# Gorilla-Lab-SCUT/GeoA3

Hardware: AMD Instinct MI355X
Metric: attack-iterations/sec (B=250, N=1024) (higher is better)
Workload: dtype f32; 1 GPU; configs[1]: PointNet 1024-pt, 250 instances sharded over 1 GPU(s) (250 on rank 0), full GeoA3 (CE + CD 1.0 + HD 0.1 + curvature 1.0 k=16), untargeted; instances_per_gpu=250, global_batch=250, npoint=1024, knn=16, classes=40, wide_mode=f16x2, presteps=150, parallelism=instance-sharded x1

## Files before the change

geoa3_amd/csrc/pointnet_wide_bwdconv.hip:

```cpp
#include "pointnet_kernels.h"
#include <type_traits>

namespace {

constexpr int WM_CI = 128;

constexpr int BW2_WAVES = 8, BW2_THREADS = 64 * BW2_WAVES;
#ifdef GEOA3_BC_STAMPS
__device__ unsigned long long g_bc_stamps[3 * 8 * 16];
#define BC_STAMP(i)                                                                                          \
  do {                                                                                                       \
    if (tid == 0 && blockIdx.x == 5 && (blockIdx.y & 31) == 7 && blockIdx.y < 256)                            \
      g_bc_stamps[((TAPS == 3 ? 2 : (GF ? 1 : 0)) * 8 + (blockIdx.y >> 5)) * 16 + (i)] = __builtin_amdgcn_s_memtime(); \
  } while (0)
#else
#define BC_STAMP(i)
#endif
constexpr int BC_PT = WM_CI + 4;
template <int TAPS, bool GF = false, bool PRE = false>
__device__ __forceinline__ void wide_bwd_conv_body(const WideBwdArgs& a) {
  extern __shared__ __attribute__((aligned(16))) float smem[];
  constexpr int COLS = 64;
  float* s_acc = smem;
  int* s_flat = reinterpret_cast<int*>(smem);
  float* s_fg = smem + a.Co * TAPS;
  const int region = max(COLS * BC_PT, 2 * a.Co * TAPS);
  using list_t = typename std::conditional<TAPS == 1, uint16_t, int>::type;
  constexpr int LSH = TAPS == 1 ? 10 : 16;
  list_t* s_list = reinterpret_cast<list_t*>(smem + region);
  int* s_off = reinterpret_cast<int*>(smem + region) + (PRE ? 0 : (TAPS == 1 ? a.Co / 2 : a.Co * TAPS));
  int* s_wcnt = s_off + COLS + 1;
  int* s_sidecol = s_wcnt + BW2_WAVES + 1;
  float* s_side = reinterpret_cast<float*>(s_sidecol + BW2_WAVES);
  float* s_mx = s_side + BW2_WAVES * WM_CI;
  const int tid = threadIdx.x, lane = tid & 63, b = blockIdx.y, m0 = blockIdx.x * COLS;
  const int wave = __builtin_amdgcn_readfirstlane(tid >> 6);
  unsigned long long gw2 = 0ull;
  if (!GF && wave < 4) gw2 = a.Zmask2[((size_t)b * ((a.N + 63) >> 6) + blockIdx.x) * 64 + lane];
  const int tiles = (a.N + 63) >> 6;
  const ulonglong2 mkw = reinterpret_cast<const ulonglong2*>(a.Zmask + ((size_t)b * tiles + blockIdx.x) * WM_CI)[lane];
  const int qt = wave & 1, qc = (wave >> 1) & 1;

  float4* s_w1 = reinterpret_cast<float4*>((reinterpret_cast<uintptr_t>(s_side) + 15) & ~(uintptr_t)15);
  const float* gb = a.g + (size_t)b * a.Co;
  const int* argb = a.arg + (size_t)b * a.Co;
  const unsigned long long lt = (1ull << lane) - 1ull;
  BC_STAMP(0);
  constexpr int U = 8;
  const int* seg = nullptr;
  int ev0 = 0;
  if constexpr (PRE) {
    const int* ho = a.hoff + (size_t)b * (a.N + 1);
    const int h0 = ho[m0], h1 = ho[min(m0 + COLS, a.N)], hv = ho[min(m0 + min(tid, COLS), a.N)];
    seg = a.hits + (size_t)b * a.Co * TAPS + h0;
    {
      const int tot = h1 - h0, per = (tot + BW2_WAVES - 1) / BW2_WAVES;
      const int lo = min(tot, wave * per), hi = min(tot, lo + per);
      if (lo < hi) ev0 = seg[min(lo + (lane & (U - 1)), hi - 1)];
    }
    for (int e = tid; e < COLS * BC_PT; e += BW2_THREADS) s_acc[e] = 0.f;
    if (tid <= COLS) s_off[tid] = hv - h0;
    BC_STAMP(1);
    __syncthreads();
    BC_STAMP(2);
  } else {
  if (tid <= COLS) s_off[tid] = 0;
  __syncthreads();
  {
  const int cpw = (a.Co + BW2_WAVES - 1) / BW2_WAVES, c_lo = wave * cpw, c_hi = min(a.Co, c_lo + cpw);
  constexpr int MAXCH = 2;
  float gch[MAXCH];
  int bch[MAXCH];
  const bool regs = cpw <= 64 * MAXCH;
#pragma unroll
  for (int ch = 0; ch < MAXCH; ++ch) {
    const int co = c_lo + 64 * ch + lane;
    const bool in = regs && co < c_hi;
    gch[ch] = in ? gb[co] : 0.f;
    bch[ch] = (in ? argb[co] : 0) - TAPS / 2 - m0;
  }
  {
    int cnt = 0;
    int chn = 0;
    for (int c0 = c_lo; c0 < c_hi; c0 += 64, ++chn) {
      const int co = c0 + lane;
      const bool in = co < c_hi;
      const float g = regs ? (chn == 0 ? gch[0] : gch[1]) : (in ? gb[co] : 0.f);
      const int base = regs ? (chn == 0 ? bch[0] : bch[1]) : ((in ? argb[co] : 0) - TAPS / 2 - m0);
#pragma unroll
      for (int tap = 0; tap < TAPS; ++tap) {
        const int c = base + tap;
        const bool hit = g != 0.f && c >= 0 && c < COLS && m0 + c < a.N;
        cnt += __popcll(__ballot(hit));
        if (hit) atomicAdd(&s_off[c], 1);
      }
    }
    if (lane == 0) s_wcnt[wave] = cnt;
  }
  __syncthreads();
  if (tid == 0) {
    int run = 0;
    for (int w = 0; w < BW2_WAVES; ++w) {
      const int c = s_wcnt[w];
      s_wcnt[w] = run;
      run += c;
    }
    s_wcnt[BW2_WAVES] = run;
  }
  if (tid >= 64 && tid < 128) {
    const int cnt = s_off[lane];
    int incl = cnt;
#pragma unroll
    for (int o = 1; o < 64; o <<= 1) {
      const int v = __shfl_up(incl, o, 64);
      if (lane >= o) incl += v;
    }
    s_off[lane] = incl - cnt;
    if (lane == 63) s_off[COLS] = incl;
  }
  __syncthreads();
  {
    int pos = s_wcnt[wave];
    int chn = 0;
    for (int c0 = c_lo; c0 < c_hi; c0 += 64, ++chn) {
      const int co = c0 + lane;
      const bool in = co < c_hi;
      const float g = regs ? (chn == 0 ? gch[0] : gch[1]) : (in ? gb[co] : 0.f);
      const int base = regs ? (chn == 0 ? bch[0] : bch[1]) : ((in ? argb[co] : 0) - TAPS / 2 - m0);
#pragma unroll
      for (int tap = 0; tap < TAPS; ++tap) {
        const int c = base + tap;
        const bool hit = g != 0.f && c >= 0 && c < COLS && m0 + c < a.N;
        const unsigned long long mask = __ballot(hit);
        if (hit) {
          const int slot = pos + __popcll(mask & lt);
          s_flat[slot] = (co * TAPS + tap) | (c << 16);
          s_fg[slot] = g;
        }
        pos += __popcll(mask);
      }
    }
  }
  __syncthreads();
  }
  const int total = s_off[COLS];
  {
    int basec[COLS / BW2_WAVES];
#pragma unroll
    for (int j = 0; j < COLS / BW2_WAVES; ++j) basec[j] = s_off[(COLS / BW2_WAVES) * wave + j];
    for (int i0 = 0; i0 < total; i0 += 64) {
      const int i = i0 + lane;
      const int e = i < total ? s_flat[i] : -1;
      const int col = e >> 16;
#pragma unroll
      for (int j = 0; j < COLS / BW2_WAVES; ++j) {
        const bool mine = col == (COLS / BW2_WAVES) * wave + j;
        const unsigned long long mask = __ballot(mine);
        if (mine) {
          const int slot = basec[j] + __popcll(mask & lt);
          s_list[slot] = TAPS == 1 ? (list_t)((e & 0xffff) | ((e >> 16) << LSH)) : (list_t)e;
        }
        basec[j] += __popcll(mask);
      }
    }
  }
  __syncthreads();
  for (int e = tid; e < COLS * BC_PT; e += BW2_THREADS) s_acc[e] = 0.f;
  __syncthreads();
  }
  const int total = s_off[COLS];
  {
    const int per = (total + BW2_WAVES - 1) / BW2_WAVES;
    const int lo = min(total, wave * per), hi = min(total, lo + per);
    const int ldW = a.ldW ? a.ldW : WM_CI;
    int cur = -1;
    float acc0 = 0.f, acc1 = 0.f;
    auto load_ev = [&](int h0) -> int {
      const int i = min(h0 + (lane & (U - 1)), hi - 1);
      if constexpr (PRE) return seg[i];
      else return (int)s_list[i];
    };
    auto dec = [&](int e) -> int {
      if constexpr (PRE) return (e & 0xffff) | (((e >> 16) - m0) << LSH);
      else return e;
    };
    int evn = 0;
    if (lo < hi) evn = PRE ? ev0 : load_ev(lo);
    int side_col = -1;
    if (lo < hi) {
      const int c0 = dec(__builtin_amdgcn_readlane(evn, 0)) >> LSH;
      if (lo > s_off[c0]) side_col = c0;
    }
    bool in_side = side_col >= 0;
    auto flush = [&]() {
      if (cur < 0) return;
      if (in_side) {
        s_side[wave * WM_CI + 2 * lane] = acc0;
        s_side[wave * WM_CI + 2 * lane + 1] = acc1;
        in_side = false;
      } else {
        *reinterpret_cast<float2*>(s_acc + cur * BC_PT + 2 * lane) = make_float2(acc0, acc1);
      }
    };
    for (int h0 = lo; h0 < hi; h0 += U) {
      float2 w[U];
      float gg[U];
      int cc[U];
      const int ev = evn;
      if (h0 + U < hi) evn = load_ev(h0 + U);
#pragma unroll
      for (int u = 0; u < U; ++u) {
        const bool ok = h0 + u < hi;
        const int e = dec(__builtin_amdgcn_readlane(ev, u));
        const int er = e & ((1 << LSH) - 1);
        w[u] = *reinterpret_cast<const float2*>(a.W + (size_t)er * ldW + 2 * lane);
        gg[u] = ok ? gb[er / TAPS] : 0.f;
        cc[u] = ok ? e >> LSH : -2;
      }
#pragma unroll
      for (int u = 0; u < U; ++u) {
        if (cc[u] == -2) break;
        if (cc[u] != cur) {
          flush();
          cur = cc[u];
          acc0 = 0.f;
          acc1 = 0.f;
        }
        acc0 += w[u].x * gg[u];
        acc1 += w[u].y * gg[u];
      }
    }
    flush();
    if (lane == 0) s_sidecol[wave] = side_col;
    BC_STAMP(3);
  }
  __syncthreads();
  BC_STAMP(4);
  if (tid < WM_CI) {
    for (int w = 1; w < BW2_WAVES; ++w) {
      const int c = s_sidecol[w];
      if (c >= 0) s_acc[c * BC_PT + tid] += s_side[w * WM_CI + tid];
    }
  }
  __syncthreads();
  BC_STAMP(5);
  if (GF && tid < 64) s_w1[tid] = make_float4(a.w1[3 * tid], a.w1[3 * tid + 1], a.w1[3 * tid + 2], a.b1[tid]);
  float tv[16];
  {
    float mx = 0.f;
#pragma unroll
    for (int j = 0; j < 8; ++j) {
      const int c = 8 * wave + j;
      const float2 v = *reinterpret_cast<const float2*>(s_acc + c * BC_PT + 2 * lane);
      const bool in = m0 + c < a.N;
      tv[2 * j] = ((mkw.x >> c) & 1ull) && in ? v.x : 0.f;
      tv[2 * j + 1] = ((mkw.y >> c) & 1ull) && in ? v.y : 0.f;
      mx = fmaxf(mx, fmaxf(__builtin_fabsf(tv[2 * j]), __builtin_fabsf(tv[2 * j + 1])));
    }
    mx = wave_max(mx);
    if (lane == 0) s_mx[wave] = mx;
  }
  __syncthreads();
  BC_STAMP(6);
  float tm = s_mx[0];
#pragma unroll
  for (int w = 1; w < BW2_WAVES; ++w) tm = fmaxf(tm, s_mx[w]);
  const unsigned Ex = sf_exp(tm);
  const float sx = sf_scale(Ex);
  constexpr int BC_PH = 2 * BC_PT;
  _Float16* s_img = reinterpret_cast<_Float16*>(s_acc);
#pragma unroll
  for (int j = 0; j < 8; ++j) {
    const float x0 = tv[2 * j] * sx, x1 = tv[2 * j + 1] * sx;
    const _Float16 h0 = (_Float16)x0, h1 = (_Float16)x1;
    _Float16* row = s_img + (8 * wave + j) * BC_PH + 2 * lane;
    *reinterpret_cast<half2v*>(row) = half2v{h0, h1};
    *reinterpret_cast<half2v*>(row + WM_CI) = half2v{(_Float16)(x0 - (float)h0), (_Float16)(x1 - (float)h1)};
  }
  __syncthreads();
  if (wave >= 4) return;
  f32x16 acc;
#pragma unroll
  for (int r = 0; r < 16; ++r) acc[r] = 0.f;
  const _Float16* brow = s_img + (32 * qc + (lane & 31)) * BC_PH + (lane >> 5) * 8;
  {
    const half8* wf = reinterpret_cast<const half8*>(a.W2th) + (size_t)qt * 8 * 2 * 64 + lane;
    constexpr int WQ = 2;
    half8 wq[WQ][2];
#pragma unroll
    for (int c = 0; c + 1 < WQ; ++c) {
      wq[c][0] = wf[(2 * c) * 64];
      wq[c][1] = wf[(2 * c + 1) * 64];
    }
#pragma unroll
    for (int c = 0; c < 8; ++c) {
      if (c + WQ - 1 < 8) {
        wq[(c + WQ - 1) % WQ][0] = wf[(2 * (c + WQ - 1)) * 64];
        wq[(c + WQ - 1) % WQ][1] = wf[(2 * (c + WQ - 1) + 1) * 64];
      }
      const half8 wh = wq[c % WQ][0], wl = wq[c % WQ][1];
      const half8 xh = *reinterpret_cast<const half8*>(brow + c * 16);
      const half8 xl = *reinterpret_cast<const half8*>(brow + WM_CI + c * 16);
      acc = __builtin_amdgcn_mfma_f32_32x32x16_f16(wh, xh, acc, 0, 0, 0);
      acc = __builtin_amdgcn_mfma_f32_32x32x16_f16(wh, xl, acc, 0, 0, 0);
      acc = __builtin_amdgcn_mfma_f32_32x32x16_f16(wl, xh, acc, 0, 0, 0);
    }
  }
  BC_STAMP(7);
  const float un = sf_unscale(Ex) * a.w2th_unscale;
  const int col = 32 * qc + (lane & 31), m = m0 + col;
  if constexpr (GF) {
    const int ln = (int)__builtin_amdgcn_mbcnt_hi(~0u, __builtin_amdgcn_mbcnt_lo(~0u, 0u));
    const int mq = m0 + 32 * qc + (ln & 31);
    const bool in = mq < a.N;
    const float* xp = a.x3 + (size_t)b * 3 * a.N + (in ? mq : a.N - 1);
    const float x0 = xp[0], x1 = xp[a.N], x2 = xp[2 * (size_t)a.N];
    float q0 = 0.f, q1 = 0.f, q2 = 0.f;
#pragma unroll
    for (int r = 0; r < 16; ++r) {
      const float4 w = s_w1[32 * qt + (r & 3) + 8 * (r >> 2) + 4 * (ln >> 5)];
      const float o = (w.x * x0 + w.y * x1 + w.z * x2 + w.w) > 0.f ? acc[r] * un : 0.f;
      q0 += w.x * o;
      q1 += w.y * o;
      q2 += w.z * o;
    }
    q0 += __shfl_xor(q0, 32, 64);
    q1 += __shfl_xor(q1, 32, 64);
    q2 += __shfl_xor(q2, 32, 64);
    float4* s_q = s_w1 + 64;
    __syncthreads();
    if (qt == 1 && ln < 32) s_q[qc * 32 + ln] = make_float4(q0, q1, q2, 0.f);
    __syncthreads();
    if (qt == 0 && ln < 32 && in) {
      const float4 o = s_q[qc * 32 + ln];
      float* dxp = a.dx3 + (size_t)b * 3 * a.N + mq;
      dxp[0] += q0 + o.x;
      dxp[a.N] += q1 + o.y;
      dxp[2 * (size_t)a.N] += q2 + o.z;
    }
    BC_STAMP(8);
    return;
  }
  float* Y = a.dY + (size_t)b * a.sYb + m;
#pragma unroll
  for (int r = 0; r < 16; ++r) {
    const int rr = 32 * qt + (r & 3) + 8 * (r >> 2);
    const unsigned g0 = qc ? (unsigned)__builtin_amdgcn_readlane((int)(unsigned)(gw2 >> 32), rr)
                           : (unsigned)__builtin_amdgcn_readlane((int)(unsigned)gw2, rr);
    const unsigned g1 = qc ? (unsigned)__builtin_amdgcn_readlane((int)(unsigned)(gw2 >> 32), rr + 4)
                           : (unsigned)__builtin_amdgcn_readlane((int)(unsigned)gw2, rr + 4);
    const unsigned gsel = lane < 32 ? g0 : g1;
    const int row = rr + 4 * (lane >> 5);
    if (m < a.N) Y[(size_t)row * a.ldY] = (gsel >> (lane & 31)) & 1u ? acc[r] * un : 0.f;
  }
  BC_STAMP(8);
}

template <int TAPS, bool PRE>
__global__ __launch_bounds__(BW2_THREADS) void wide_bwd_conv_kernel(WideBwdArgs a) {
  wide_bwd_conv_body<TAPS, false, PRE>(a);
}
template <bool PRE>
__global__ __launch_bounds__(BW2_THREADS) __attribute__((amdgpu_waves_per_eu(8, 8))) void wide_bwd_conv_first_kernel(WideBwdArgs a) {
  wide_bwd_conv_body<1, true, PRE>(a);
}

}

#ifdef GEOA3_BC_STAMPS
extern "C" int geoa3_debug_bc_stamps(unsigned long long* out) {
  return hipMemcpyFromSymbol(out, HIP_SYMBOL(g_bc_stamps), sizeof(g_bc_stamps)) == hipSuccess ? 0 : -1;
}
#endif
int launch_wide_bwd_conv(const WideBwdArgs& a, hipStream_t s) {
  const bool gf = a.dx3 != nullptr;
  if ((a.taps != 1 && a.taps != 3) || !a.Zmask || !a.W2th || a.Co * a.taps > 0xffff || (a.taps == 1 && a.Co > 1024) ||
      (gf ? (!a.x3 || !a.w1 || !a.b1 || a.taps != 1) : (!a.Zmask2 || !a.dY)))
    return GEOA3_ENOSUPPORT;
  dim3 grid((a.N + 63) / 64, a.B);
  const size_t region = (size_t)64 * BC_PT > 2 * (size_t)a.Co * a.taps ? (size_t)64 * BC_PT : 2 * (size_t)a.Co * a.taps;
  const bool pre = a.hits && a.hoff;
  const size_t lds = (region + (pre ? 0 : (a.taps == 1 ? (size_t)a.Co / 2 : (size_t)a.Co * a.taps)) + 65 + 2 * BW2_WAVES + 1 + BW2_WAVES * WM_CI + 16 + 3 + 4) * sizeof(float);
  auto go = [&](auto kern) {
    (void)hipFuncSetAttribute(reinterpret_cast<const void*>(kern), hipFuncAttributeMaxDynamicSharedMemorySize, (int)lds);
    hipLaunchKernelGGL(kern, grid, dim3(BW2_THREADS), lds, s, a);
  };
  if (a.taps == 1 && a.dx3) pre ? go(wide_bwd_conv_first_kernel<true>) : go(wide_bwd_conv_first_kernel<false>);
  else if (a.taps == 1) pre ? go(wide_bwd_conv_kernel<1, true>) : go(wide_bwd_conv_kernel<1, false>);
  else pre ? go(wide_bwd_conv_kernel<3, true>) : go(wide_bwd_conv_kernel<3, false>);
  GEOA3_CHECK_LAUNCH();
  return GEOA3_OK;
}
```

Measured before the change: 650.4 iterations/s of a 250-instance batch.

## Software-pipeline backward-conv hit gathers and prefetch MFMA weights before barriers

The scatter-accumulate loop now loads 64 hit events per lane at once, gathers their gradient values in one load, and double-buffers the weight-row fetches in groups of 8 so loads overlap the accumulation. W2th MFMA operands, the Zmask2 word, the x3 coordinates and the w1 weights are prefetched before the reduction barriers, and the prefetch depth grows to 3 with sched_barrier ordering. The dx3 read is hoisted ahead of the reduction, and the non-first kernel gets waves_per_eu(8,8). This hides global-memory latency behind the barriers and compute, at the cost of more live registers that the occupancy attribute could force into spills.

```diff
diff --git a/geoa3_amd/csrc/pointnet_wide_bwdconv.hip b/geoa3_amd/csrc/pointnet_wide_bwdconv.hip
--- a/geoa3_amd/csrc/pointnet_wide_bwdconv.hip
+++ b/geoa3_amd/csrc/pointnet_wide_bwdconv.hip
@@ -35,20 +35,22 @@
   float* s_mx = s_side + BW2_WAVES * WM_CI;
   const int tid = threadIdx.x, lane = tid & 63, b = blockIdx.y, m0 = blockIdx.x * COLS;
   const int wave = __builtin_amdgcn_readfirstlane(tid >> 6);
-  unsigned long long gw2 = 0ull;
-  if (!GF && wave < 4) gw2 = a.Zmask2[((size_t)b * ((a.N + 63) >> 6) + blockIdx.x) * 64 + lane];
   const int tiles = (a.N + 63) >> 6;
   const ulonglong2 mkw = reinterpret_cast<const ulonglong2*>(a.Zmask + ((size_t)b * tiles + blockIdx.x) * WM_CI)[lane];
   const int qt = wave & 1, qc = (wave >> 1) & 1;
 
-  float4* s_w1 = reinterpret_cast<float4*>((reinterpret_cast<uintptr_t>(s_side) + 15) & ~(uintptr_t)15);
+  float4* s_w1 = reinterpret_cast<float4*>(smem + (((int)(s_side - smem) + 3) & ~3));
   const float* gb = a.g + (size_t)b * a.Co;
   const int* argb = a.arg + (size_t)b * a.Co;
   const unsigned long long lt = (1ull << lane) - 1ull;
   BC_STAMP(0);
-  constexpr int U = 8;
+  constexpr int U = 8, NB = 2, CH = 64;
   const int* seg = nullptr;
   int ev0 = 0;
+  float4 w1v = make_float4(0.f, 0.f, 0.f, 0.f);
+  if constexpr (GF) {
+    if (tid < 64) w1v = make_float4(a.w1[3 * tid], a.w1[3 * tid + 1], a.w1[3 * tid + 2], a.b1[tid]);
+  }
   if constexpr (PRE) {
     const int* ho = a.hoff + (size_t)b * (a.N + 1);
     const int h0 = ho[m0], h1 = ho[min(m0 + COLS, a.N)], hv = ho[min(m0 + min(tid, COLS), a.N)];
@@ -56,7 +58,7 @@
     {
       const int tot = h1 - h0, per = (tot + BW2_WAVES - 1) / BW2_WAVES;
       const int lo = min(tot, wave * per), hi = min(tot, lo + per);
-      if (lo < hi) ev0 = seg[min(lo + (lane & (U - 1)), hi - 1)];
+      if (lo < hi) ev0 = seg[min(lo + lane, hi - 1)];
     }
     for (int e = tid; e < COLS * BC_PT; e += BW2_THREADS) s_acc[e] = 0.f;
     if (tid <= COLS) s_off[tid] = hv - h0;
@@ -175,8 +177,8 @@
     const int ldW = a.ldW ? a.ldW : WM_CI;
     int cur = -1;
     float acc0 = 0.f, acc1 = 0.f;
-    auto load_ev = [&](int h0) -> int {
-      const int i = min(h0 + (lane & (U - 1)), hi - 1);
+    auto load_ev = [&](int c0) -> int {
+      const int i = min(c0 + lane, hi - 1);
       if constexpr (PRE) return seg[i];
       else return (int)s_list[i];
     };
@@ -202,49 +204,80 @@
         *reinterpret_cast<float2*>(s_acc + cur * BC_PT + 2 * lane) = make_float2(acc0, acc1);
       }
     };
-    for (int h0 = lo; h0 < hi; h0 += U) {
-      float2 w[U];
-      float gg[U];
-      int cc[U];
-      const int ev = evn;
-      if (h0 + U < hi) evn = load_ev(h0 + U);
-#pragma unroll
-      for (int u = 0; u < U; ++u) {
-        const bool ok = h0 + u < hi;
-        const int e = dec(__builtin_amdgcn_readlane(ev, u));
-        const int er = e & ((1 << LSH) - 1);
-        w[u] = *reinterpret_cast<const float2*>(a.W + (size_t)er * ldW + 2 * lane);
-        gg[u] = ok ? gb[er / TAPS] : 0.f;
-        cc[u] = ok ? e >> LSH : -2;
-      }
-#pragma unroll
-      for (int u = 0; u < U; ++u) {
-        if (cc[u] == -2) break;
-        if (cc[u] != cur) {
-          flush();
-          cur = cc[u];
-          acc0 = 0.f;
-          acc1 = 0.f;
+    for (int c0 = lo; c0 < hi; c0 += CH) {
+      const int ed = dec(evn);
+      const float gv = gb[(ed & ((1 << LSH) - 1)) / TAPS];
+      if (c0 + CH < hi) evn = load_ev(c0 + CH);
+      float2 w[NB][U];
+      auto request = [&](int k, float2 (&wk)[U]) {
+#pragma unroll
+        for (int u = 0; u < U; ++u) {
+          const int er = __builtin_amdgcn_readlane(ed, U * k + u) & ((1 << LSH) - 1);
+          wk[u] = *reinterpret_cast<const float2*>(a.W + (size_t)er * ldW + 2 * lane);
         }
-        acc0 += w[u].x * gg[u];
-        acc1 += w[u].y * gg[u];
+      };
+      auto consume = [&](int k, const float2 (&wk)[U]) {
+#pragma unroll
+        for (int u = 0; u < U; ++u) {
+          if (c0 + U * k + u >= hi) break;
+          const int c = __builtin_amdgcn_readlane(ed, U * k + u) >> LSH;
+          const float g = __int_as_float(__builtin_amdgcn_readlane(__float_as_int(gv), U * k + u));
+          if (c != cur) {
+            flush();
+            cur = c;
+            acc0 = 0.f;
+            acc1 = 0.f;
+          }
+          acc0 += wk[u].x * g;
+          acc1 += wk[u].y * g;
+        }
+      };
+#pragma unroll
+      for (int k = 0; k < CH / U + NB - 1; ++k) {
+        if (k < CH / U && c0 + U * k < hi) request(k, w[k % NB]);
+        if (k >= NB - 1) {
+          const int j = k - (NB - 1);
+          if (c0 + U * j >= hi) break;
+          consume(j, w[j % NB]);
+        }
       }
     }
     flush();
     if (lane == 0) s_sidecol[wave] = side_col;
     BC_STAMP(3);
   }
+  constexpr int WQ = 3;
+  const half8* wf = reinterpret_cast<const half8*>(a.W2th) + (size_t)qt * 8 * 2 * 64 + lane;
+  half8 wq[WQ][2];
+  unsigned long long gw2 = 0ull;
+  float x0 = 0.f, x1 = 0.f, x2 = 0.f;
+  if (wave < 4) {
+    if constexpr (!GF) gw2 = a.Zmask2[((size_t)b * tiles + blockIdx.x) * 64 + lane];
+#pragma unroll
+    for (int c = 0; c < WQ; ++c) {
+      wq[c][0] = wf[(2 * c) * 64];
+      wq[c][1] = wf[(2 * c + 1) * 64];
+    }
+    if constexpr (GF) {
+      const float* xp = a.x3 + (size_t)b * 3 * a.N + min(m0 + 32 * qc + (lane & 31), a.N - 1);
+      x0 = xp[0], x1 = xp[a.N], x2 = xp[2 * (size_t)a.N];
+    }
+  }
   __syncthreads();
   BC_STAMP(4);
   if (tid < WM_CI) {
+    int sc[BW2_WAVES];
+#pragma unroll
+    for (int w = 1; w < BW2_WAVES; ++w) sc[w] = s_sidecol[w];
+#pragma unroll
     for (int w = 1; w < BW2_WAVES; ++w) {
-      const int c = s_sidecol[w];
+      const int c = sc[w];
       if (c >= 0) s_acc[c * BC_PT + tid] += s_side[w * WM_CI + tid];
     }
   }
   __syncthreads();
   BC_STAMP(5);
-  if (GF && tid < 64) s_w1[tid] = make_float4(a.w1[3 * tid], a.w1[3 * tid + 1], a.w1[3 * tid + 2], a.b1[tid]);
+  if (GF && tid < 64) s_w1[tid] = w1v;
   float tv[16];
   {
     float mx = 0.f;
@@ -278,32 +311,24 @@
     *reinterpret_cast<half2v*>(row + WM_CI) = half2v{(_Float16)(x0 - (float)h0), (_Float16)(x1 - (float)h1)};
   }
   __syncthreads();
+  BC_STAMP(9);
   if (wave >= 4) return;
   f32x16 acc;
 #pragma unroll
   for (int r = 0; r < 16; ++r) acc[r] = 0.f;
   const _Float16* brow = s_img + (32 * qc + (lane & 31)) * BC_PH + (lane >> 5) * 8;
-  {
-    const half8* wf = reinterpret_cast<const half8*>(a.W2th) + (size_t)qt * 8 * 2 * 64 + lane;
-    constexpr int WQ = 2;
-    half8 wq[WQ][2];
-#pragma unroll
-    for (int c = 0; c + 1 < WQ; ++c) {
-      wq[c][0] = wf[(2 * c) * 64];
-      wq[c][1] = wf[(2 * c + 1) * 64];
-    }
-#pragma unroll
-    for (int c = 0; c < 8; ++c) {
-      if (c + WQ - 1 < 8) {
-        wq[(c + WQ - 1) % WQ][0] = wf[(2 * (c + WQ - 1)) * 64];
-        wq[(c + WQ - 1) % WQ][1] = wf[(2 * (c + WQ - 1) + 1) * 64];
-      }
-      const half8 wh = wq[c % WQ][0], wl = wq[c % WQ][1];
-      const half8 xh = *reinterpret_cast<const half8*>(brow + c * 16);
-      const half8 xl = *reinterpret_cast<const half8*>(brow + WM_CI + c * 16);
-      acc = __builtin_amdgcn_mfma_f32_32x32x16_f16(wh, xh, acc, 0, 0, 0);
-      acc = __builtin_amdgcn_mfma_f32_32x32x16_f16(wh, xl, acc, 0, 0, 0);
-      acc = __builtin_amdgcn_mfma_f32_32x32x16_f16(wl, xh, acc, 0, 0, 0);
+#pragma unroll
+  for (int c = 0; c < 8; ++c) {
+    const half8 wh = wq[c % WQ][0], wl = wq[c % WQ][1];
+    const half8 xh = *reinterpret_cast<const half8*>(brow + c * 16);
+    const half8 xl = *reinterpret_cast<const half8*>(brow + WM_CI + c * 16);
+    acc = __builtin_amdgcn_mfma_f32_32x32x16_f16(wh, xh, acc, 0, 0, 0);
+    acc = __builtin_amdgcn_mfma_f32_32x32x16_f16(wh, xl, acc, 0, 0, 0);
+    acc = __builtin_amdgcn_mfma_f32_32x32x16_f16(wl, xh, acc, 0, 0, 0);
+    if (c + WQ < 8) {
+      wq[c % WQ][0] = wf[(2 * (c + WQ)) * 64];
+      wq[c % WQ][1] = wf[(2 * (c + WQ) + 1) * 64];
+      __builtin_amdgcn_sched_barrier(0);
     }
   }
   BC_STAMP(7);
@@ -313,8 +338,9 @@
     const int ln = (int)__builtin_amdgcn_mbcnt_hi(~0u, __builtin_amdgcn_mbcnt_lo(~0u, 0u));
     const int mq = m0 + 32 * qc + (ln & 31);
     const bool in = mq < a.N;
-    const float* xp = a.x3 + (size_t)b * 3 * a.N + (in ? mq : a.N - 1);
-    const float x0 = xp[0], x1 = xp[a.N], x2 = xp[2 * (size_t)a.N];
+    float* dxp = a.dx3 + (size_t)b * 3 * a.N + (in ? mq : a.N - 1);
+    const float d0 = dxp[0], d1 = dxp[a.N], d2 = dxp[2 * (size_t)a.N];
+    __builtin_amdgcn_sched_barrier(0);
     float q0 = 0.f, q1 = 0.f, q2 = 0.f;
 #pragma unroll
     for (int r = 0; r < 16; ++r) {
@@ -333,10 +359,9 @@
     __syncthreads();
     if (qt == 0 && ln < 32 && in) {
       const float4 o = s_q[qc * 32 + ln];
-      float* dxp = a.dx3 + (size_t)b * 3 * a.N + mq;
-      dxp[0] += q0 + o.x;
-      dxp[a.N] += q1 + o.y;
-      dxp[2 * (size_t)a.N] += q2 + o.z;
+      dxp[0] = d0 + (q0 + o.x);
+      dxp[a.N] = d1 + (q1 + o.y);
+      dxp[2 * (size_t)a.N] = d2 + (q2 + o.z);
     }
     BC_STAMP(8);
     return;
@@ -357,7 +382,7 @@
 }
 
 template <int TAPS, bool PRE>
-__global__ __launch_bounds__(BW2_THREADS) void wide_bwd_conv_kernel(WideBwdArgs a) {
+__global__ __launch_bounds__(BW2_THREADS) __attribute__((amdgpu_waves_per_eu(8, 8))) void wide_bwd_conv_kernel(WideBwdArgs a) {
   wide_bwd_conv_body<TAPS, false, PRE>(a);
 }
 template <bool PRE>
```

After: 657.8 iterations/s of a 250-instance batch, median of 6. 1.1% higher.
